# Stylish-TTS/stylish-tts

Hardware: AMD Instinct MI355X
Metric: audio frames/sec/GPU (24 kHz) forward+backward; DDP scaling 1/2/4/8 MI355X (higher is better)
Workload: dtype bf16 GEMM operands, f32 accumulation/storage; 1 GPU; c3: B=32/GPU T=520 frames (6.5 s) L=100

## Files before the change

include/stylish_hip.h:

```cpp
#ifndef STYLISH_HIP_H
#define STYLISH_HIP_H

#include <stddef.h>
#include <stdint.h>

#ifdef __cplusplus
extern "C" {
#endif

typedef enum {
  STY_OK = 0,
  STY_EINVAL = -1,
  STY_ESHAPE = -2,
  STY_EHIP = -3,
  STY_ENOMEM = -4,
  STY_ESTATE = -5
} sty_status;

typedef struct sty_model sty_model;

int sty_version(void);
const char *sty_last_error(void);

int sty_model_create(const char *kind, sty_model **out);
// ... 87 lines not shown
int sty_ctc_loss_fwd_bwd(int B, int T, int V1, int U, const float *log_probs, const float *log_priors, float prior_scale,
                         const int64_t *targets, const int64_t *input_lengths, const int64_t *target_lengths, int blank,
                         float weight, double *nll, float *loss, int32_t *status, float *d_logits, void *workspace,
                         size_t ws_bytes, void *stream);

int sty_convnext_fwd(sty_model *m, const char *prefix, int B, int C, int T, const float *x, const float *style,
                     float *y, void *workspace, size_t ws_bytes, void *stream);
int sty_resblock_fwd(sty_model *m, const char *prefix, int B, int T, const float *x, const float *style, float *y,
                     void *workspace, size_t ws_bytes, void *stream);
int sty_block_train_workspace_bytes(sty_model *m, const char *kind, const char *prefix, int B, int C, int T,
                                    size_t *bytes);
int sty_block_fwd_bwd(sty_model *m, const char *kind, const char *prefix, int B, int C, int T, const float *x,
                      const float *style, const float *gy, float *y, float *gx, float *d_style, void *workspace,
                      size_t ws_bytes, void *stream);
int sty_attention_workspace_bytes(int B, int H, int T, size_t *bytes);
int sty_attention_fwd_bwd(int B, int H, int DH, int T, const float *q, const float *k, const float *v,
                          const int64_t *lengths, const float *d_o, float *o, float *dq, float *dk, float *dv,
                          void *workspace, size_t ws_bytes, void *stream);
int sty_stft64_fwd(int B, int N, const float *wave, float *spec, float *phase, void *stream);
void sty_stft64_bases_host(float *out);
int sty_istft64_fwd(int B, int F, const float *logamp, const float *real, const float *imag, float *audio,
                    void *stream);
int sty_source_fwd(int B, int T, const float *pitch, const float *voiced, const float *noise, uint64_t seed,
                   const float *lin_w, const float *lin_b, float *prior, void *workspace, size_t ws_bytes,
                   void *stream);
int sty_source_workspace_bytes(int B, int T, size_t *bytes);
int sty_grn_bwd_workspace_bytes(int B, int C4, int T, size_t *bytes);
int sty_grn_bwd(int B, int C4, int T, const float *h, const float *ds, const float *gamma, int from_gx, float *coef,
                float *dgamma, void *workspace, size_t ws_bytes, void *stream);
int sty_act_bwd(int kind, int B, int C, int T, const float *x, float *dy, const float *alpha, const float *h,
                const float *coef, int fused, float *dx, int accumulate, float *dalpha, void *stream);
int sty_adain_finalize(int B, int C, int T, int nseg, const double *part, const float *gb, float eps, float *a, float *s,
                       float *mean, float *rstd, void *stream);

int sty_model_enable_training(sty_model *m);
typedef struct {
  int bn_batch_stats;
  int sn_power_iter;
  int f0_smooth;
  int energy_smooth;
  float bn_momentum;
  unsigned dropout_seed;
  float text_dropout;
  int compute_bf16;
  int frozen;
  float block_dropout;
} sty_train_opts;
int sty_model_set_train_opts(sty_model *m, const sty_train_opts *opts);

typedef void (*sty_grad_hook)(void *user, int segment);
int sty_model_set_grad_hook(sty_model *m, sty_grad_hook hook, void *user);
int sty_model_bind_grad(sty_model *m, const char *key, float *grad);
int sty_vocoder_train_workspace_bytes(sty_model *m, int B, int T, size_t *bytes);
int sty_vocoder_fwd_train(sty_model *m, const sty_vocoder_io *io, void *workspace, size_t ws_bytes, void *stream);
int sty_vocoder_bwd(sty_model *m, const float *d_audio, float *d_mel, float *d_style, void *stream);
int sty_speech_train_workspace_bytes(sty_model *m, int B, int L, int T, size_t *bytes);
int sty_speech_fwd_train(sty_model *m, const sty_speech_io *io, void *workspace, size_t ws_bytes, void *stream);
int sty_speech_bwd(sty_model *m, const float *d_audio, float *d_style, float *d_energy, void *stream);
int sty_speech_prepare_train(sty_model *m, void *stream);
int sty_speech_bwd_pe(sty_model *m, const float *d_audio, float *d_style, float *d_pitch, float *d_energy, void *stream);
int sty_speech_d_style_ready(sty_model *m, void *stream);
int sty_speech_branch_stream(sty_model *m, void **stream);
int sty_style_train_workspace_bytes(sty_model *m, int B, int T, size_t *bytes);
int sty_style_fwd_train(sty_model *m, int B, int T, const float *mel, float *style, void *workspace, size_t ws_bytes,
                        void *stream);
int sty_style_bwd(sty_model *m, const float *d_style, void *stream);
// ... 163 lines not shown
```

stylish_tts_amd/csrc/api.hip:

```cpp
#include <math.h>
#include <stdarg.h>
#include <string.h>
#include <stdlib.h>
#include <cxxabi.h>

#include <algorithm>
#include <functional>
#include <map>
#include <mutex>
#include <string>
#include <tuple>

#include "model.h"

namespace sty {

static thread_local char g_err[1024] = "";
void set_error(const char* fmt, ...) {
  va_list ap;
  va_start(ap, fmt);
  vsnprintf(g_err, sizeof(g_err), fmt, ap);
  va_end(ap);
}
int hip_fail(hipError_t e, const char* what) {
// ... 3380 lines not shown
  return launch_grn_bwd(from_gx ? gx : nullptr, part, nseg, gamma, ds, B, C4, coef, dgamma, st);
}
int sty_act_bwd(int kind, int B, int C, int T, const float* x, float* dy, const float* alpha, const float* h,
                const float* coef, int fused, float* dx, int accumulate, float* dalpha, void* stream) {
  if (!x || !dy || !dx || B <= 0 || C <= 0 || T <= 0 || (kind == ACT_SNAKE && !alpha) || ((h != nullptr) != (coef != nullptr))) {
    set_error("sty_act_bwd: bad argument");
    return STY_EINVAL;
  }
  hipStream_t st = S(stream);
  if (h && !fused) {
    const int rc = launch_row_scale_add(h, coef, 0.f, B * C, T, dy, st);
    if (rc) return rc;
    h = coef = nullptr;
  }
  if (deterministic_mode() && kind == ACT_SNAKE && dalpha && B > 1) {
    for (int b = 0; b < B; ++b) {
      const size_t o = (size_t)b * C * T;
      const int rc = launch_act_bwd(kind, x + o, dy + o, alpha, 1, C, T, dx + o, accumulate, dalpha, st, h ? h + o : nullptr,
                                    coef ? coef + (size_t)b * C : nullptr);
      if (rc) return rc;
    }
    return STY_OK;
  }
  return launch_act_bwd(kind, x, dy, alpha, B, C, T, dx, accumulate, dalpha, st, h, coef);
}
int sty_adain_finalize(int B, int C, int T, int nseg, const double* part, const float* gb, float eps, float* a, float* s,
                       float* mean, float* rstd, void* stream) {
  if (!part || !gb || !a || !s || B <= 0 || C <= 0 || T <= 0 || nseg <= 0 || ((mean != nullptr) != (rstd != nullptr))) {
    set_error("sty_adain_finalize: bad argument");
    return STY_EINVAL;
  }
  return launch_adain_finalize(part, nseg, gb, B, C, T, eps, a, s, S(stream), mean, rstd);
}
int sty_mel_workspace_bytes(int B, int N, int n_fft, int hop, size_t* bytes) {
  if (!bytes || B <= 0 || N <= n_fft / 2 || n_fft <= 0 || hop <= 0) {
    set_error("sty_mel_workspace_bytes: bad argument");
    return STY_EINVAL;
  }
  *bytes = mel_workspace_floats(B, N, n_fft, hop, 80) * sizeof(float);
  return STY_OK;
}
int sty_mel_fwd(int B, int N, const float* audio, int n_fft, int win_length, int hop, float mean, float std_,
                float* mel, float* energy, void* workspace, size_t ws_bytes, void* stream) {
  if (!audio || !mel || !workspace || B <= 0 || N <= n_fft / 2 || win_length > n_fft || hop <= 0 || std_ == 0.f) {
    set_error("sty_mel_fwd: bad argument");
    return STY_EINVAL;
  }
  if (ws_bytes < mel_workspace_floats(B, N, n_fft, hop, 80) * sizeof(float)) {
    set_error("sty_mel_fwd: workspace too small");
    return STY_ENOMEM;
  }
  return launch_mel(B, N, audio, n_fft, win_length, hop, 80, 24000, mean, std_, mel, energy, (float*)workspace,
                    S(stream));
}
int sty_multispec_workspace_bytes(int B, int N, size_t* bytes) {
  if (!bytes || B <= 0 || N <= 1024) {
    set_error("sty_multispec_workspace_bytes: bad argument");
    return STY_EINVAL;
  }
  size_t mx = 0;
  const int res[3][2] = {{512, 128}, {1024, 256}, {2048, 512}};
  for (auto& r : res) {
    const size_t n = multispec_workspace_floats(B, N, r[0], r[1]);
    mx = n > mx ? n : mx;
  }
  *bytes = mx * sizeof(float);
// ... 105 lines not shown
```

stylish_tts_amd/csrc/conv2d.hip:

```cpp
#include <stdlib.h>

#include "weights.h"

namespace sty {

constexpr int SN_SLICES = 8;
size_t sn_power_iter_scratch_floats(int Cout, int n) { return (size_t)SN_SLICES * n + Cout; }

int sn_wtu_blocks(int n) { return SN_SLICES * ((n + 255) / 256); }
__device__ __forceinline__ int snj_n(const SnPrepJob& j) { return j.depthwise ? 9 : j.Cin * j.KH * j.K; }
__global__ __launch_bounds__(256) void sn_wt_u_multi_kernel(const SnPrepJob* __restrict__ jobs, const int* __restrict__ job_of_blk) {
  const SnPrepJob j = jobs[job_of_blk[blockIdx.x]];
  const int n = snj_n(j), nib = (n + 255) / 256;
  const int local = (int)blockIdx.x - j.wtu0, slice = local / nib, i = (local - slice * nib) * 256 + threadIdx.x;
  if (i >= n) return;
  float s = 0.f;
  for (int co = slice; co < j.Cout; co += SN_SLICES) s = fmaf(j.w[(size_t)co * n + i], j.u[co], s);
  j.power[(size_t)slice * n + i] = s;
}
__global__ __launch_bounds__(256) void sn_normalize_multi_kernel(const SnPrepJob* __restrict__ jobs, int which) {
  __shared__ double red[256];
  const SnPrepJob j = jobs[blockIdx.x];
  const int nv = snj_n(j);
  const int n = which ? j.Cout : nv, slices = which ? 1 : SN_SLICES;
// ... 186 lines not shown
  return STY_OK;
}

__global__ __launch_bounds__(256) void dwconv2d_s2_kernel(const float* __restrict__ x, const float* __restrict__ w9,
                                                          const float* __restrict__ bias, int C, int H, int W, int Ho,
                                                          int Wo, float* __restrict__ y, __bf16* __restrict__ y16) {
  const int ldi = W + 1, ldo = Wo + 1;
  const int i = blockIdx.x * 256 + threadIdx.x;
  if (i >= Ho * ldo) return;
  const int ho = i / ldo, wo = i - ho * ldo;
  const int bc = blockIdx.y, c = bc % C;
  float* out = y + (size_t)bc * Ho * ldo + i;
  __bf16* out16 = y16 ? y16 + (size_t)bc * Ho * ldo + i : nullptr;
  if (wo == Wo) {
    *out = 0.f;
    if (out16) *out16 = (__bf16)0.f;
    return;
  }
  const float* p = x + (size_t)bc * H * ldi;
  float acc = bias[c];
#pragma unroll
  for (int kh = 0; kh < 3; ++kh) {
    const int hi = 2 * ho + kh - 1;
    if (hi < 0 || hi >= H) continue;
#pragma unroll
    for (int kw = 0; kw < 3; ++kw) {
      const int wi = 2 * wo + kw - 1;
      if (wi >= 0 && wi < W) acc = fmaf(w9[c * 9 + kh * 3 + kw], p[(size_t)hi * ldi + wi], acc);
    }
  }
  *out = acc;
  if (out16) *out16 = (__bf16)(acc < 0.f ? 0.2f * acc : acc);
}
int launch_dwconv2d_s2(const float* x, const float* w9, const float* bias, int B, int C, int H, int W, float* y,
                       hipStream_t st, __bf16* y16_lrelu) {
  const int Ho = (H - 1) / 2 + 1, Wo = (W - 1) / 2 + 1;
  hipLaunchKernelGGL(dwconv2d_s2_kernel, dim3(cdiv(Ho * (Wo + 1), 256), B * C), dim3(256), 0, st, x, w9, bias, C, H, W, Ho,
                     Wo, y, y16_lrelu);
  STY_LAUNCH_CHECK();
  return STY_OK;
}

__global__ __launch_bounds__(256) void avgpool2_kernel(const float* __restrict__ x, int H, int W, int Ho, int Wo,
                                                       float scale, float* __restrict__ y, __bf16* __restrict__ y16) {
  const int ldi = W + 1, ldo = Wo + 1;
  const int i = blockIdx.x * 256 + threadIdx.x;
  if (i >= Ho * ldo) return;
  const int ho = i / ldo, wo = i - ho * ldo;
  const int bc = blockIdx.y;
  float* out = y + (size_t)bc * Ho * ldo + i;
  __bf16* out16 = y16 ? y16 + (size_t)bc * Ho * ldo + i : nullptr;
  if (wo == Wo) {
    *out = 0.f;
    if (out16) *out16 = (__bf16)0.f;
    return;
  }
  const float* p = x + (size_t)bc * H * ldi;
  const int w0 = 2 * wo, w1 = min(2 * wo + 1, W - 1);
  const float s = p[(size_t)(2 * ho) * ldi + w0] + p[(size_t)(2 * ho) * ldi + w1] +
                  p[(size_t)(2 * ho + 1) * ldi + w0] + p[(size_t)(2 * ho + 1) * ldi + w1];
  *out = s * 0.25f * scale;
  if (out16) *out16 = (__bf16)(s * 0.25f * scale);
}
int launch_avgpool2(const float* x, int BC, int H, int W, float scale, float* y, hipStream_t st, __bf16* y16) {
  const int Ho = H / 2, Wo = (W + 1) / 2;
  hipLaunchKernelGGL(avgpool2_kernel, dim3(cdiv(Ho * (Wo + 1), 256), BC), dim3(256), 0, st, x, H, W, Ho, Wo, scale, y, y16);
  STY_LAUNCH_CHECK();
  return STY_OK;
}

__global__ __launch_bounds__(1024) void pool_fc_kernel(const float* __restrict__ x, int C, int n, float inv_count,
// ... 52 lines not shown
  const float* p = x + (size_t)bc * n;
  float* d = dx + (size_t)bc * n;
  __bf16* d16 = dx16 ? dx16 + (size_t)bc * n : nullptr;
  const float* mk = mask16 ? mask16 + (size_t)(bc / C) * n : nullptr;
  float wk[9];
#pragma unroll
  for (int k = 0; k < 9; ++k) wk[k] = w9[c * 9 + k];
  float wacc[10];
#pragma unroll
  for (int k = 0; k < 10; ++k) wacc[k] = 0.f;
  const int nq = Ho * Wo;
  auto put = [&](int o, float v) {
    if (ACC) v += d[o];
    if (ACC || dx) d[o] = v;
    if (!ACC && d16) d16[o] = (__bf16)(v * mk[o]);
  };
#pragma unroll 1
  for (int rr = 0; rr < DW2_R; ++rr) {
    const int q = (blockIdx.x * DW2_R + rr) * 256 + threadIdx.x;
    if (q >= nq) break;
    const int qh = q / Wo, qw = q - qh * Wo;
    const bool w1 = qw + 1 < Wo, h1 = qh + 1 < Ho;
    auto G = [&](int ho, int wo, bool ok) {
      if (!ok) return 0.f;
      float v = g[(size_t)ho * ldo + wo];
      if (gt && !(gt[(size_t)ho * ldo + wo] > 0.f)) v *= 0.2f;
      return v;
    };
    const float G00 = G(qh, qw, true), G01 = G(qh, qw + 1, w1), G10 = G(qh + 1, qw, h1), G11 = G(qh + 1, qw + 1, w1 && h1);
    const int hi = 2 * qh, wi = 2 * qw;
    const bool c1 = wi + 1 < W, r1 = hi + 1 < H;
    const int o0 = hi * ldi + wi, o1 = o0 + ldi;
    const float xee = p[o0], xeo = c1 ? p[o0 + 1] : 0.f, xoe = r1 ? p[o1] : 0.f, xoo = (c1 && r1) ? p[o1 + 1] : 0.f;
    put(o0, wk[4] * G00);
    wacc[4] = fmaf(G00, xee, wacc[4]);
    wacc[9] += G00;
    if (c1) {
      put(o0 + 1, fmaf(wk[3], G01, wk[5] * G00));
      wacc[3] = fmaf(G01, xeo, wacc[3]);
      wacc[5] = fmaf(G00, xeo, wacc[5]);
    }
    if (r1) {
      put(o1, fmaf(wk[1], G10, wk[7] * G00));
      wacc[1] = fmaf(G10, xoe, wacc[1]);
      wacc[7] = fmaf(G00, xoe, wacc[7]);
      if (c1) {
        put(o1 + 1, fmaf(wk[0], G11, fmaf(wk[2], G10, fmaf(wk[6], G01, wk[8] * G00))));
        wacc[0] = fmaf(G11, xoo, wacc[0]);
        wacc[2] = fmaf(G10, xoo, wacc[2]);
        wacc[6] = fmaf(G01, xoo, wacc[6]);
        wacc[8] = fmaf(G00, xoo, wacc[8]);
      }
    }
    if (qw == Wo - 1) {
      put(hi * ldi + W, 0.f);
      if (r1) put((hi + 1) * ldi + W, 0.f);
    }
  }
  const int lane = threadIdx.x & 63, wave = threadIdx.x >> 6;
#pragma unroll
  for (int k = 0; k < 10; ++k) {
    float v = wacc[k];
    for (int o = 32; o > 0; o >>= 1) v += __shfl_xor(v, o);
    if (lane == 0) red[wave][k] = v;
  }
  __syncthreads();
  if (threadIdx.x < 10) {
    const int k = threadIdx.x;
    part[((size_t)bc * gridDim.x + blockIdx.x) * 10 + k] = (red[0][k] + red[1][k]) + (red[2][k] + red[3][k]);
  }
}
__global__ __launch_bounds__(64) void dwconv2d_s2_bwd_w_sum_kernel(const float* __restrict__ part, int C, int B, int nblk,
                                                                   float* __restrict__ dw9, float* __restrict__ db) {
  const int c = blockIdx.x, lane = threadIdx.x;
  float s[10];
#pragma unroll
  for (int k = 0; k < 10; ++k) s[k] = 0.f;
  for (int b = 0; b < B; ++b) {
    const float* pp = part + ((size_t)(b * C + c) * nblk) * 10;
    for (int j = lane; j < nblk; j += 64)
#pragma unroll
      for (int k = 0; k < 10; ++k) s[k] += pp[(size_t)j * 10 + k];
  }
#pragma unroll
  for (int k = 0; k < 10; ++k) {
    float v = s[k];
    for (int o = 32; o > 0; o >>= 1) v += __shfl_xor(v, o);
    s[k] = v;
  }
  if (lane == 0) {
#pragma unroll
    for (int k = 0; k < 9; ++k) dw9[c * 9 + k] += s[k];
    if (db) db[c] += s[9];
  }
}
size_t dwconv2d_s2_bwd_scratch_floats(int B, int C, int H, int W) { return (size_t)B * C * cdiv(H * (W + 1), 1024) * 10; }
int launch_dwconv2d_s2_bwd(const float* x, const float* gy, const float* gate, const float* w9, int B, int C, int H, int W,
                           float* dx, int accumulate, float* dw9, float* db, float* scratch, hipStream_t st, __bf16* dx16,
                           const float* mask16) {
  const int Ho = (H - 1) / 2 + 1, Wo = (W - 1) / 2 + 1;
  const int nblk = cdiv(Ho * Wo, 256 * DW2_R);
  if (dx16 && (accumulate || !mask16)) {
    set_error("dwconv2d_s2_bwd: the operand twin of dx needs the overwriting form and the mask");
    return STY_EINVAL;
  }
  if (!dx && !dx16) {
    set_error("dwconv2d_s2_bwd: neither dx nor its operand twin to write");
    return STY_EINVAL;
  }
  if (accumulate)
    hipLaunchKernelGGL(dwconv2d_s2_bwd_kernel<true>, dim3(nblk, B * C), dim3(256), 0, st, x, gy, gate, w9, C, H, W, Ho, Wo, dx,
                       scratch, nullptr, nullptr);
  else
    hipLaunchKernelGGL(dwconv2d_s2_bwd_kernel<false>, dim3(nblk, B * C), dim3(256), 0, st, x, gy, gate, w9, C, H, W, Ho, Wo, dx,
                       scratch, dx16, mask16);
  hipLaunchKernelGGL(dwconv2d_s2_bwd_w_sum_kernel, dim3(C), dim3(64), 0, st, scratch, C, B, nblk, dw9, db);
  STY_LAUNCH_CHECK();
  return STY_OK;
}
__global__ void dw2d_sn_unpack_kernel(const float* __restrict__ g9, const float* __restrict__ w,
                                      const float* __restrict__ u, const float* __restrict__ v,
                                      const float* __restrict__ t, int C, float* __restrict__ dW) {
  __shared__ float red[2][256];
  float sig = 0.f, dot = 0.f;
  for (int i = threadIdx.x; i < C; i += 256) sig += t[i];
  for (int i = threadIdx.x; i < C * 9; i += 256) dot = fmaf(g9[i], w[i], dot);
  red[0][threadIdx.x] = sig;
  red[1][threadIdx.x] = dot;
  __syncthreads();
  for (int o = 128; o > 0; o >>= 1) {
    if (threadIdx.x < o) {
      red[0][threadIdx.x] += red[0][threadIdx.x + o];
      red[1][threadIdx.x] += red[1][threadIdx.x + o];
    }
    __syncthreads();
  }
  const float inv = 1.0f / red[0][0], k = red[1][0] * inv * inv;
  for (int i = threadIdx.x; i < C * 9; i += 256) dW[i] += g9[i] * inv - k * u[i / 9] * v[i % 9];
}
int launch_dw2d_sn_unpack(const float* g9, const float* w, const float* u, const float* v, const float* t, int C,
                          float* dW, hipStream_t st) {
  hipLaunchKernelGGL(dw2d_sn_unpack_kernel, dim3(1), dim3(256), 0, st, g9, w, u, v, t, C, dW);
  STY_LAUNCH_CHECK();
  return STY_OK;
}
__global__ __launch_bounds__(256) void avgpool2_bwd_kernel(const float* __restrict__ gy, int H, int W, int Ho, int Wo,
                                                           float scale, float* __restrict__ dx,
// ... 133 lines not shown
```

stylish_tts_amd/csrc/model.h:

```cpp
#pragma once
#include <math.h>

#include <map>
#include <string>
#include <unordered_map>
#include <vector>

#include "sty_common.h"
#include "weights.h"

namespace sty {

struct Param {
  const float* p = nullptr;
  std::vector<int64_t> shape;
};

int convnext32_ntiles(int T);
int launch_convnext32(const Cnx32Args& a, int B, int pass, hipStream_t st);
int launch_attention(const AttnArgs& a, int B, int DH, hipStream_t st);
int launch_rope_n(float* q, float* k, int B, int H, int DH, int L, int d, hipStream_t st, float sgn = 1.0f);
int launch_style_expand(const float* style, int B, int S, int L, float* y, hipStream_t st);
int launch_row_sum_add(const float* src, int rows, int L, float* dst, hipStream_t st);
int launch_wn_dw_bwd(const float* dw, const float* g, const float* v, int C, int K, float* dg, float* dv, hipStream_t st);
// ... 33 lines not shown
                 size_t ws_bytes, hipStream_t st, size_t* need);
struct AcousticGan {
  const sty_specdisc_params* p[3] = {nullptr, nullptr, nullptr};
  const sty_specdisc_grads* g[3] = {nullptr, nullptr, nullptr};
  float w_gen = 1.f, disc_scale = 1.f;
  float* out = nullptr;
  int bf16 = 0;
  void* ws = nullptr;
  size_t ws_bytes = 0;
};
size_t acoustic_gan_workspace_bytes(int B, int N, int with_grads);
int launch_acoustic_loss_gan(int B, int N, const float* audio_gt, const float* audio_pred, float w_mel, float w_phase,
                             float* losses_out, float* d_pred, float* ws, const AcousticGan* gan, hipStream_t st);
int launch_multispec_single(int B, int N, const float* audio, int n_fft, int hop, int sample_rate, float* mag,
                            float* phase, float* fft_mag, float* ws, hipStream_t st);
size_t loss_features_scratch_floats(int B, int N);
int launch_loss_features(int B, int N, const float* audio, int r, float* mag, float* scratch, hipStream_t st);

struct Bump {
  char* base = nullptr;
  size_t off = 0, cap = 0;
  bool overflow = false;
  template <typename T>
  T* take(size_t n) {
    off = align_up(off, 256);
    T* p = base ? reinterpret_cast<T*>(base + off) : nullptr;
    off += n * sizeof(T);
    if (base && off > cap) overflow = true;
    return p;
  }
};

int launch_dwconv2d_s2(const float* x, const float* w9, const float* bias, int B, int C, int H, int W, float* y,
                       hipStream_t st, __bf16* y16_lrelu = nullptr);
int launch_avgpool2(const float* x, int BC, int H, int W, float scale, float* y, hipStream_t st, __bf16* y16 = nullptr);
int launch_pool_fc(const float* x, int B, int C, int n, int count, const float* W, const float* bvec, int S,
                   float* out, hipStream_t st);
struct AdaFc {
  int idx = -1;
  int C = 0;
  size_t off = 0;
};

struct ConvNeXt {
  int C = 0;
  const float *dw_w = nullptr, *dw_b = nullptr, *b1 = nullptr, *alpha = nullptr, *grn_gamma = nullptr;
  AdaFc norm;
  PackedConv pw1, pw2;
  const float* w2a = nullptr;
  const float* w1p = nullptr;
  const float *w1_raw = nullptr, *w2_raw = nullptr;
};

struct ResBlock32 {
  PackedConv c1[3], c2[3];
  AdaFc n1[3], n2[3];
  const float *a1[3], *a2[3];
};

struct Conformer {
  AdaFc ff1n, ff2n, attn_n, conv_n, post_n;
  PackedConv ff1a, ff1b, ff2a, ff2b, to_q, to_kv, to_out, pw1, pw2;
  const float *dw_w, *dw_b, *bn_w, *bn_b, *bn_rm, *bn_rv;
};

struct VocoderPlan {
  PackedConv amp_input_conv;
// ... 271 lines not shown
int style_fc_bwd_slots(int nlayers);
int launch_istft64_bwd(int B, int F, const float* audio, const float* daudio, const float* logamp, const float* real,
                       const float* imag, const float* bbr, const float* bbi, float* dlogamp, float* dreal,
                       float* dimag, hipStream_t st);
size_t wgrad_partial_floats(const PackedConv& w, int B, int T);
struct WgReduceDefer;
WgReduceDefer* wgrad_defer_create();
void wgrad_defer_destroy(WgReduceDefer* d);
WgReduceDefer* wgrad_defer_set(WgReduceDefer* d);
size_t wgrad_defer_pending(const WgReduceDefer* d);
int wgrad_defer_flush(WgReduceDefer* d, int site, hipStream_t st);
void launch_wgrad_reduce_planes(const float* partial, int nslices, size_t plane, size_t stride, int nb, float* gwp,
                                float* gbias, hipStream_t st);
int launch_attention_bwd(const AttnArgs& a, const float* dO, float* dQ, float* dK, float* dV, size_t dqbs, size_t dkbs,
                         size_t dvbs, size_t dobs, int B, int DH, float* ws, hipStream_t st, int overwrite = 0);
bool attention_bwd_can_overwrite(const AttnArgs& a, int DH);
bool attention_bwd_mfma_dh(int DH);
size_t attention_bwd_ws_floats(int B, int H, int T);
int launch_rope_signed(float* q, float* k, int B, int H, int DH, int L, int d, const float* theta4, float sgn,
                       hipStream_t st);
int launch_embedding_bwd(const int64_t* tokens, const float* g, int B, int L, int H, int ntok, float scale, float* demb,
                         hipStream_t st, bool det = false);
int launch_bmm_ct_bwd(const float* g, const float* ali, int B, int C, int L, int T, float* denc, hipStream_t st);
int launch_slice_add(const float* src, int Csrc, int c0, int B, int C, int T, float* dst, hipStream_t st);
int launch_fnv_bwd(const float* pitch, const float* energy, const float* voiced, const float* w34, const float* g, int B,
                   int T, float* dw34, float* dp, float* de, float* dv, hipStream_t st, bool det = false);
int fnv_bwd_slices();
int launch_fnv_unpack(const float* dw34, const float* g0, const float* v0, const float* g1, const float* v1,
                      const float* g2, const float* v2, float* dg0, float* dv0, float* db0, float* dg1, float* dv1,
                      float* db1, float* dg2, float* dv2, float* db2, hipStream_t st);
size_t dwconv2d_s2_bwd_scratch_floats(int B, int C, int H, int W);
int launch_dwconv2d_s2_bwd(const float* x, const float* gy, const float* gate, const float* w9, int B, int C, int H, int W, float* dx,
                           int accumulate, float* dw9, float* db, float* scratch, hipStream_t st, __bf16* dx16 = nullptr,
                           const float* mask16 = nullptr);
int launch_pad_cols(const float* x, size_t rows, int W, float* y, hipStream_t st);
int launch_flat_mask(int B, int H, int Wp, int Hv, int Wv, float* m, hipStream_t st);
int launch_dw2d_sn_unpack(const float* g9, const float* w, const float* u, const float* v, const float* t, int C,
                          float* dW, hipStream_t st);
int launch_avgpool2_bwd(const float* gy, int BC, int H, int W, float scale, float* dx, const float* gate, hipStream_t st,
                        __bf16* dx16 = nullptr, const float* mask16 = nullptr, int C = 0);
int launch_pool_fc_bwd(const float* x, int B, int C, int n, int count, const float* W, int S, const float* gs,
                       float* dW, float* db, float* dx, int accumulate, hipStream_t st, float* det_a = nullptr);
int launch_bn_train_fwd(const float* x, const float* w, const float* b, float* rm, float* rv, float eps, float momentum,
                        int B, int C, int T, float* y, float* mean, float* rstd, double* part, hipStream_t st);
int launch_bn_train_bwd(const float* x, const float* dy, const float* w, const float* mean, const float* rstd, int B,
                        int C, int T, float* dx, int accumulate, float* dw, float* db, float* sums, hipStream_t st);
int launch_dropout(const float* x, const float* res, size_t n, float p, unsigned seed, unsigned site, float* y,
                   int accumulate, hipStream_t st, size_t group = 1);
int launch_box_smooth(const float* x, int B, int T, int width, float* y, int accumulate, hipStream_t st);
size_t sn_power_iter_scratch_floats(int Cout, int n);
int trainer_style_forward(struct Trainer* t, int B, int T, const float* mel, float* style, void* ws, size_t ws_bytes,
                          hipStream_t st, size_t* need, const float* pitch = nullptr, const float* energy = nullptr);
int trainer_style_backward(struct Trainer* t, const float* d_style, hipStream_t st);
int trainer_style_tap(struct Trainer* t, int i, int grad, float* dst, int* C, int* H, int* W, hipStream_t st);
inline sty_vocoder_io vocoder_io_of(const sty_speech_io& io) {
  sty_vocoder_io v = io.voc_taps;
  v.B = io.B;
  v.T = io.T;
  v.style = io.style;
  v.pitch = io.denormal_pitch;
  v.voiced = io.voiced;
  v.noise = io.noise;
  v.prior_override = io.prior_override;
  v.seed = io.seed;
  v.audio = io.audio;
  return v;
}
// ... 25 lines not shown
```

stylish_tts_amd/lib.py:

```python
import ctypes as C
import os

os.environ.setdefault("GPU_MAX_HW_QUEUES", "2")

HERE = os.path.dirname(os.path.abspath(__file__))
LIB_PATH = os.path.join(HERE, "libstylish_hip.so")


class StyError(RuntimeError):
    status = None


class StyDeviceError(StyError):
    """STY_EHIP: the HIP runtime reported an error (a failed launch, copy or allocation, a sticky device fault, no device).
    Not a refusal: nothing may be launched behind it, so nobody who skips refused work may catch it as one (`refused_on_host`)."""


STY_EHIP = -3


def refused_on_host(e):
    return isinstance(e, StyError) and not isinstance(e, StyDeviceError) and e.status != STY_EHIP


# ... 73 lines not shown
    "sty_model_set_train_opts": (C.c_int, [_P, C.POINTER(TrainOpts)]),
    "sty_vocoder_train_workspace_bytes": (C.c_int, [_P, _I, _I, _SZP]),
    "sty_vocoder_fwd_train": (C.c_int, [_P, C.POINTER(VocoderIO), _P, C.c_size_t, _P]),
    "sty_vocoder_bwd": (C.c_int, [_P, _P, _P, _P, _P]),
    "sty_speech_train_workspace_bytes": (C.c_int, [_P, _I, _I, _I, _SZP]),
    "sty_speech_fwd_train": (C.c_int, [_P, C.POINTER(SpeechIO), _P, C.c_size_t, _P]),
    "sty_speech_bwd": (C.c_int, [_P, _P, _P, _P, _P]),
    "sty_speech_prepare_train": (C.c_int, [_P, _P]),
    "sty_speech_bwd_pe": (C.c_int, [_P, _P, _P, _P, _P, _P]),
    "sty_speech_d_style_ready": (C.c_int, [_P, _P]),
    "sty_speech_branch_stream": (C.c_int, [_P, C.POINTER(C.c_void_p)]),
    "sty_style_train_workspace_bytes": (C.c_int, [_P, _I, _I, _SZP]),
    "sty_style_fwd_train": (C.c_int, [_P, _I, _I, _P, _P, _P, C.c_size_t, _P]),
    "sty_style_prepare_train": (C.c_int, [_P, _P]),
    "sty_style_bwd": (C.c_int, [_P, _P, _P]),
    "sty_style_tap": (C.c_int, [_P, _I, _I, _P, C.POINTER(C.c_int), C.POINTER(C.c_int), C.POINTER(C.c_int), _P]),
    "sty_duration_workspace_bytes": (C.c_int, [_P, _I, _I, _SZP]),
    "sty_duration_fwd": (C.c_int, [_P, _I, _I, _P, _P, _P, _P, _P, C.c_size_t, _P]),
    "sty_pitch_energy_workspace_bytes": (C.c_int, [_P, _I, _I, _I, _SZP]),
    "sty_pitch_energy_fwd": (C.c_int, [_P, _I, _I, _I, _P, _P, _P, _P, _P, _P, _P, C.c_size_t, _P]),
    "sty_pitch_style_workspace_bytes": (C.c_int, [_P, _I, _I, _SZP]),
    "sty_pitch_style_fwd": (C.c_int, [_P, _I, _I, _P, _P, _P, _P, _P, C.c_size_t, _P]),
    "sty_conv1d_workspace_bytes": (C.c_int, [_I, _I, _I, _SZP]),
    "sty_conv1d_fwd": (C.c_int, [_I, _I, _I, _I, _I, _I, _P, _P, _P, _P, _P, C.c_size_t, _I, _P]),
    "sty_conv1d_fwd_ex": (C.c_int, [_I, _I, _I, _I, _I, _I, _P, _P, _P, _P, _P, _P, _I, _I, _P, _P, C.c_size_t, _I, _P]),
    "sty_conv1d_route": (C.c_int, [_I, _I, _I, _I, _I, _I, _I, _I, C.POINTER(C.c_int)]),
    "sty_conv1d_bwd_workspace_bytes": (C.c_int, [_I, _I, _I, _I, _I, _SZP]),
    "sty_conv1d_bwd": (C.c_int, [_I, _I, _I, _I, _I, _I, _P, _P, _P, _P, _P, _P, _P, C.c_size_t, _I, _P]),
    "sty_partial_sum": (C.c_int, [_I, _P, _I, _I, _I, _P, _P, _P]),
    "sty_grn_bwd_workspace_bytes": (C.c_int, [_I, _I, _I, _SZP]),
    "sty_grn_bwd": (C.c_int, [_I, _I, _I, _P, _P, _P, _I, _P, _P, _P, C.c_size_t, _P]),
    "sty_act_bwd": (C.c_int, [_I, _I, _I, _I, _P, _P, _P, _P, _P, _I, _P, _I, _P, _P]),
    "sty_adain_finalize": (C.c_int, [_I, _I, _I, _I, _P, _P, C.c_float, _P, _P, _P, _P, _P]),
    "sty_adamw_step": (C.c_int, [C.c_size_t, _P, _P, _P, _P, C.c_float, C.c_float, C.c_float, C.c_float, C.c_float,
                                 _I, C.c_float, _P]),
    "sty_adamw_step_scaled": (C.c_int, [C.c_size_t, _P, _P, _P, _P, C.c_double, _P, C.c_float, C.c_float, C.c_float,
                                        C.c_float, _I, C.c_float, _P]),
    "sty_disc_lr_track": (C.c_int, [_P, _P, C.c_double, C.c_double, C.c_double, C.c_double, C.c_double, _P]),
    "sty_model_set_grad_hook": (C.c_int, [_P, _P, _P]),
    "sty_acoustic_loss_workspace_bytes": (C.c_int, [_I, _I, _SZP]),
    "sty_acoustic_loss_target": (C.c_int, [_I, _I, _P, _P, C.c_size_t, _P]),
    "sty_acoustic_loss_fwd_bwd": (C.c_int, [_I, _I, _P, _P, C.c_float, C.c_float, _P, _P, _P, C.c_size_t, _P]),
    "sty_mel_loss_workspace_bytes": (C.c_int, [_I, _I, _SZP]),
    "sty_mel_loss_features": (C.c_int, [_I, _I, _I, _I, _SZP, C.POINTER(C.c_int)]),
    "sty_mel_loss_fwd": (C.c_int, [_I, _I, _P, _P, _P, _P, _P, C.c_size_t, _P]),
    "sty_pitch_loss_fwd": (C.c_int, [_I, _I, _P, _P, _P, _P, C.c_size_t, _P]),
    "sty_duration_loss_fwd": (C.c_int, [_I, _I, _I, _P, _P, _P, _P, _P, _P, _P, _P, C.c_size_t, _P]),
    "sty_specdisc_workspace_bytes": (C.c_int, [_I, _I, _I, _I, _SZP]),
    "sty_specdisc_forward": (C.c_int, [_P, _I, _I, _I, _P, _P, _I, _P, C.c_size_t, _P]),
    "sty_specdisc_losses": (C.c_int, [_P, _I, _I, _I, _P, _P, C.c_float, _P, _P, C.c_float, _P, _P, _I, _P, C.c_size_t,
                                      _P]),
    "sty_prediction_to_duration": (C.c_int, [_I, _I, _I, _P, _P, _P, _P, _P]),
    "sty_duration_loss_fwd_bwd": (C.c_int, [_I, _I, _I, _P, _P, _P, _P, _P, _P, C.c_float, C.c_float, _P, _P, _P, _P,
                                            C.c_size_t, _P]),
    "sty_duration_train_workspace_bytes": (C.c_int, [_P, _I, _I, _SZP]),
    "sty_duration_fwd_train": (C.c_int, [_P, _I, _I, _P, _P, _P, _P, _P, C.c_size_t, _P]),
    "sty_duration_bwd": (C.c_int, [_P, _P, _P, _P]),
    "sty_pitch_loss_fwd_bwd": (C.c_int, [_I, _I, _P, _P, C.c_float, _I, _P, _P, _P, C.c_size_t, _P]),
    "sty_pitch_energy_train_workspace_bytes": (C.c_int, [_P, _I, _I, _I, _SZP]),
    "sty_pitch_energy_fwd_train": (C.c_int, [_P, _I, _I, _I, _P, _P, _P, _P, _P, _P, _P, C.c_size_t, _P]),
    "sty_pitch_energy_bwd": (C.c_int, [_P, _P, _P, _P, _P]),
    "sty_pitch_style_train_workspace_bytes": (C.c_int, [_P, _I, _I, _SZP]),
    "sty_pitch_style_fwd_train": (C.c_int, [_P, _I, _I, _P, _P, _P, _P, _P, C.c_size_t, _P]),
    "sty_pitchdisc_workspace_bytes": (C.c_int, [_I, _I, _I, _I, _I, _SZP]),
    "sty_pitchdisc_forward": (C.c_int, [_P, _I, _I, _I, _I, _P, _P, _P, C.c_size_t, _P]),
    "sty_pitchdisc_losses": (C.c_int, [_P, _I, _I, _I, _I, _P, _P, C.c_float, _P, _P, C.c_float, _P, _P, _P, C.c_size_t,
# ... 120 lines not shown
```

Baseline: 402,700 frames/s.

## Add LDS-staged wide kernels for stride-2 depthwise conv2d forward and backward

Adds new forward and backward kernels for the stride-2 3x3 depthwise conv2d. They stage the needed input (forward) or upstream gradient (backward) rows into shared memory with vectorized float4 loads, then have each thread produce four outputs with vector stores. The backward kernel walks the input grid (gather form), computes the weight-gradient partials alongside, and reduces them across waves. It also exposes the forward and backward as C API entry points with a 'present' flag that falls back to the old kernels, plus an env-var opt-out. The new path runs only when shapes and pointers meet alignment conditions, which adds branch complexity and the risk of subtle indexing errors at boundaries.

After: 406,500 frames/s, median of 6. About the same (+0.9%).

```diff
diff --git a/include/stylish_hip.h b/include/stylish_hip.h
--- a/include/stylish_hip.h
+++ b/include/stylish_hip.h
@@ -143,6 +143,12 @@
                 const float *coef, int fused, float *dx, int accumulate, float *dalpha, void *stream);
 int sty_adain_finalize(int B, int C, int T, int nseg, const double *part, const float *gb, float eps, float *a, float *s,
                        float *mean, float *rstd, void *stream);
+int sty_dwconv2d_s2_fwd(int B, int C, int H, int W, const float *x, const float *w9, const float *bias, float *y, void *y16,
+                        int present, void *stream);
+int sty_dwconv2d_s2_bwd_workspace_bytes(int B, int C, int H, int W, size_t *bytes);
+int sty_dwconv2d_s2_bwd(int B, int C, int H, int W, const float *x, const float *gy, const float *gate, const float *w9,
+                        float *dx, int accumulate, void *dx16, const float *mask16, float *dw9, float *db, void *workspace,
+                        size_t ws_bytes, int present, void *stream);
 
 int sty_model_enable_training(sty_model *m);
 typedef struct {
diff --git a/stylish_tts_amd/csrc/api.hip b/stylish_tts_amd/csrc/api.hip
--- a/stylish_tts_amd/csrc/api.hip
+++ b/stylish_tts_amd/csrc/api.hip
@@ -3436,6 +3436,36 @@
   }
   return launch_adain_finalize(part, nseg, gb, B, C, T, eps, a, s, S(stream), mean, rstd);
 }
+int sty_dwconv2d_s2_fwd(int B, int C, int H, int W, const float* x, const float* w9, const float* bias, float* y, void* y16,
+                        int present, void* stream) {
+  if (!x || !w9 || !bias || !y || B <= 0 || C <= 0 || H <= 0 || W <= 0) {
+    set_error("sty_dwconv2d_s2_fwd: bad argument");
+    return STY_EINVAL;
+  }
+  return launch_dwconv2d_s2(x, w9, bias, B, C, H, W, y, S(stream), reinterpret_cast<__bf16*>(y16), present != 0);
+}
+int sty_dwconv2d_s2_bwd_workspace_bytes(int B, int C, int H, int W, size_t* bytes) {
+  if (!bytes || B <= 0 || C <= 0 || H <= 0 || W <= 0) {
+    set_error("sty_dwconv2d_s2_bwd_workspace_bytes: bad argument");
+    return STY_EINVAL;
+  }
+  *bytes = dwconv2d_s2_bwd_scratch_floats(B, C, H, W) * sizeof(float);
+  return STY_OK;
+}
+int sty_dwconv2d_s2_bwd(int B, int C, int H, int W, const float* x, const float* gy, const float* gate, const float* w9,
+                        float* dx, int accumulate, void* dx16, const float* mask16, float* dw9, float* db, void* workspace,
+                        size_t ws_bytes, int present, void* stream) {
+  if (!x || !gy || !w9 || !dw9 || !workspace || B <= 0 || C <= 0 || H <= 0 || W <= 0 || (accumulate && !dx)) {
+    set_error("sty_dwconv2d_s2_bwd: bad argument");
+    return STY_EINVAL;
+  }
+  if (ws_bytes < dwconv2d_s2_bwd_scratch_floats(B, C, H, W) * sizeof(float)) {
+    set_error("sty_dwconv2d_s2_bwd: workspace too small");
+    return STY_ENOMEM;
+  }
+  return launch_dwconv2d_s2_bwd(x, gy, gate, w9, B, C, H, W, dx, accumulate, dw9, db, (float*)workspace, S(stream),
+                                reinterpret_cast<__bf16*>(dx16), mask16, present != 0);
+}
 int sty_mel_workspace_bytes(int B, int N, int n_fft, int hop, size_t* bytes) {
   if (!bytes || B <= 0 || N <= n_fft / 2 || n_fft <= 0 || hop <= 0) {
     set_error("sty_mel_workspace_bytes: bad argument");
diff --git a/stylish_tts_amd/csrc/conv2d.hip b/stylish_tts_amd/csrc/conv2d.hip
--- a/stylish_tts_amd/csrc/conv2d.hip
+++ b/stylish_tts_amd/csrc/conv2d.hip
@@ -242,11 +242,104 @@
   *out = acc;
   if (out16) *out16 = (__bf16)(acc < 0.f ? 0.2f * acc : acc);
 }
+constexpr int DW2W_LD = 8;
+constexpr int DW2W_CAP = DW2W_LD * 256 * 4;
+__device__ __forceinline__ int dw2w_sw8(int i) { return i + (i >> 3); }
+__global__ __launch_bounds__(256) void dwconv2d_s2_wide_kernel(const float* __restrict__ x, const float* __restrict__ w9,
+                                                               const float* __restrict__ bias, int C, int H, int W, int Ho,
+                                                               int Wo, int npb, float* __restrict__ y,
+                                                               __bf16* __restrict__ y16) {
+  __shared__ float xs[DW2W_CAP + DW2W_CAP / 8];
+  const int ldi = W + 1, ldo = Wo + 1, no = Ho * ldo;
+  const int bc = blockIdx.y, c = bc % C, tid = threadIdx.x;
+  const int o0 = blockIdx.x * npb, o1 = min(o0 + npb, no);
+  const int ho_lo = o0 / ldo, ho_hi = (o1 - 1) / ldo;
+  const int hi_lo = max(2 * ho_lo - 1, 0), hi_hi = min(2 * ho_hi + 1, H - 1);
+  const int s0 = (hi_lo * ldi) & ~3, s1 = ((hi_hi + 1) * ldi + 3) & ~3;
+  const float* p = x + (size_t)bc * H * ldi + s0;
+  float4 v[DW2W_LD];
+#pragma unroll
+  for (int k = 0; k < DW2W_LD; ++k) {
+    const int r = (k * 256 + tid) * 4;
+    v[k] = s0 + r < s1 ? *reinterpret_cast<const float4*>(p + r) : make_float4(0.f, 0.f, 0.f, 0.f);
+  }
+#pragma unroll
+  for (int k = 0; k < DW2W_LD; ++k) {
+    const int r = (k * 256 + tid) * 4;
+    if (s0 + r < s1) {
+      float* q = xs + dw2w_sw8(r);
+      q[0] = v[k].x;
+      q[1] = v[k].y;
+      q[2] = v[k].z;
+      q[3] = v[k].w;
+    }
+  }
+  __syncthreads();
+  const int o = o0 + tid * 4;
+  if (o >= o1) return;
+  float wk[9];
+#pragma unroll
+  for (int k = 0; k < 9; ++k) wk[k] = w9[c * 9 + k];
+  const float bv = bias[c];
+  int ho = o / ldo, wo = o - ho * ldo;
+  float out[4];
+#pragma unroll
+  for (int e = 0; e < 4; ++e) {
+    float acc = 0.f;
+    if (wo < Wo) {
+      const int rc = 2 * ho * ldi - s0 + 2 * wo;
+      const bool rt = ho > 0, rb = 2 * ho + 1 < H, cl = wo > 0, cr = 2 * wo + 1 < W;
+      acc = bv;
+#pragma unroll
+      for (int kh = 0; kh < 3; ++kh)
+#pragma unroll
+        for (int kw = 0; kw < 3; ++kw) {
+          const bool ok = (kh == 0 ? rt : kh == 2 ? rb : true) && (kw == 0 ? cl : kw == 2 ? cr : true);
+          const float xv = xs[dw2w_sw8(ok ? rc + (kh - 1) * ldi + (kw - 1) : rc)];
+          acc = ok ? fmaf(wk[kh * 3 + kw], xv, acc) : acc;
+        }
+    }
+    out[e] = acc;
+    if (++wo == ldo) {
+      wo = 0;
+      ++ho;
+    }
+  }
+  *reinterpret_cast<float4*>(y + (size_t)bc * no + o) = make_float4(out[0], out[1], out[2], out[3]);
+  if (y16) {
+    typedef __bf16 bf16x4 __attribute__((ext_vector_type(4)));
+    bf16x4 h;
+#pragma unroll
+    for (int e = 0; e < 4; ++e) h[e] = (__bf16)(out[e] < 0.f ? 0.2f * out[e] : out[e]);
+    *reinterpret_cast<bf16x4*>(y16 + (size_t)bc * no + o) = h;
+  }
+}
+static bool dw2_wide_off() { return getenv("STY_NO_DW2_WIDE") != nullptr; }
+static int dw2_wide_fwd_npb(int H, int W) {
+  const int Ho = (H - 1) / 2 + 1, Wo = (W - 1) / 2 + 1, ldi = W + 1, ldo = Wo + 1;
+  if ((H * ldi) % 4 || (Ho * ldo) % 4) return 0;
+  for (int npb = 1024; npb >= 256; npb /= 2) {
+    const int rows_o = std::min(Ho, (npb - 1 + ldo - 1) / ldo + 1);
+    const int rows_i = std::min(H, 2 * rows_o + 1);
+    if ((size_t)rows_i * ldi + 6 <= (size_t)DW2W_CAP) return npb;
+  }
+  return 0;
+}
 int launch_dwconv2d_s2(const float* x, const float* w9, const float* bias, int B, int C, int H, int W, float* y,
-                       hipStream_t st, __bf16* y16_lrelu) {
+                       hipStream_t st, __bf16* y16_lrelu, bool present) {
   const int Ho = (H - 1) / 2 + 1, Wo = (W - 1) / 2 + 1;
-  hipLaunchKernelGGL(dwconv2d_s2_kernel, dim3(cdiv(Ho * (Wo + 1), 256), B * C), dim3(256), 0, st, x, w9, bias, C, H, W, Ho,
-                     Wo, y, y16_lrelu);
+  const double ni = (double)B * C * H * (W + 1), no = (double)B * C * Ho * (Wo + 1);
+  const int npb = present || dw2_wide_off() || (((size_t)x | (size_t)y) & 15) || ((size_t)y16_lrelu & 7) ? 0 : dw2_wide_fwd_npb(H, W);
+  char detail[48];
+  snprintf(detail, sizeof(detail), "c%d h%d w%d", C, H, W);
+  ProfScope prof(npb ? "dwconv2d_s2_wide_kernel" : "dwconv2d_s2_kernel", 18.0 * no, 4.0 * ni + (y16_lrelu ? 6.0 : 4.0) * no, st,
+                 detail);
+  if (npb)
+    hipLaunchKernelGGL(dwconv2d_s2_wide_kernel, dim3(cdiv(Ho * (Wo + 1), npb), B * C), dim3(256), 0, st, x, w9, bias, C, H, W,
+                       Ho, Wo, npb, y, y16_lrelu);
+  else
+    hipLaunchKernelGGL(dwconv2d_s2_kernel, dim3(cdiv(Ho * (Wo + 1), 256), B * C), dim3(256), 0, st, x, w9, bias, C, H, W, Ho,
+                       Wo, y, y16_lrelu);
   STY_LAUNCH_CHECK();
   return STY_OK;
 }
@@ -365,7 +458,10 @@
     const bool c1 = wi + 1 < W, r1 = hi + 1 < H;
     const int o0 = hi * ldi + wi, o1 = o0 + ldi;
     const float xee = p[o0], xeo = c1 ? p[o0 + 1] : 0.f, xoe = r1 ? p[o1] : 0.f, xoo = (c1 && r1) ? p[o1 + 1] : 0.f;
-    put(o0, wk[4] * G00);
+    if (ACC)
+      d[o0] = fmaf(wk[4], G00, d[o0]);
+    else
+      put(o0, wk[4] * G00);
     wacc[4] = fmaf(G00, xee, wacc[4]);
     wacc[9] += G00;
     if (c1) {
@@ -427,12 +523,186 @@
     if (db) db[c] += s[9];
   }
 }
+constexpr int DW2W_CH = 4;
+constexpr int DW2W_NI = DW2W_CH * 256 * 4;
+constexpr int DW2W_GLD = 4;
+constexpr int DW2W_GCAP = DW2W_GLD * 256 * 4;
+__device__ __forceinline__ int dw2w_sw2(int i) { return i + (i >> 1); }
+__device__ __forceinline__ void dw2w_fmac(float& acc, float a, float b) { asm("v_fmac_f32 %0, %1, %2" : "+v"(acc) : "v"(a), "v"(b)); }
+__device__ __forceinline__ void dw2w_pin(float4& v) { asm volatile("" : "+v"(v.x), "+v"(v.y), "+v"(v.z), "+v"(v.w)); }
+template <bool ACC>
+__global__ __launch_bounds__(256) void dwconv2d_s2_bwd_wide_kernel(const float* __restrict__ x, const float* __restrict__ gy,
+                                                                   const float* __restrict__ gate,
+                                                                   const float* __restrict__ w9, int C, int H, int W, int Ho,
+                                                                   int Wo, float* __restrict__ dx, float* __restrict__ part,
+                                                                   __bf16* __restrict__ dx16,
+                                                                   const float* __restrict__ mask16) {
+  __shared__ float gs[DW2W_GCAP + DW2W_GCAP / 2];
+  __shared__ float red[4][10];
+  const int bc = blockIdx.y, c = bc % C, tid = threadIdx.x;
+  const int ldi = W + 1, ldo = Wo + 1, n = H * ldi;
+  const int i0 = blockIdx.x * DW2W_NI, i1 = min(i0 + DW2W_NI, n);
+  const int ho_lo = (i0 / ldi) >> 1, ho_hi = min((((i1 - 1) / ldi) >> 1) + 1, Ho - 1);
+  const int g0 = (ho_lo * ldo) & ~3, g1 = ((ho_hi + 1) * ldo + 3) & ~3;
+  const float* g = gy + (size_t)bc * Ho * ldo + g0;
+  const float* gt = gate ? gate + (size_t)bc * Ho * ldo + g0 : nullptr;
+  const float* p = x + (size_t)bc * n;
+  float* d = dx + (size_t)bc * n;
+  __bf16* d16 = dx16 ? dx16 + (size_t)bc * n : nullptr;
+  const float* mk = mask16 ? mask16 + (size_t)(bc / C) * n : nullptr;
+  const float4 zero4 = make_float4(0.f, 0.f, 0.f, 0.f);
+  float4 gv[DW2W_GLD], tv[DW2W_GLD], xv[DW2W_CH], mv[DW2W_CH], dv[DW2W_CH];
+#pragma unroll
+  for (int k = 0; k < DW2W_GLD; ++k) {
+    const int r = (k * 256 + tid) * 4, rc = g0 + r < g1 ? r : 0;
+    gv[k] = *reinterpret_cast<const float4*>(g + rc);
+    tv[k] = zero4;
+    if (gt) tv[k] = *reinterpret_cast<const float4*>(gt + rc);
+  }
+#pragma unroll
+  for (int j = 0; j < DW2W_CH; ++j) {
+    const int i = i0 + (j * 256 + tid) * 4, ic = i < i1 ? i : i0;
+    xv[j] = *reinterpret_cast<const float4*>(p + ic);
+    mv[j] = dv[j] = zero4;
+    if (!ACC && d16) mv[j] = *reinterpret_cast<const float4*>(mk + ic);
+    if (ACC) dv[j] = *reinterpret_cast<const float4*>(d + ic);
+  }
+#pragma unroll
+  for (int k = 0; k < DW2W_GLD; ++k) {
+    dw2w_pin(gv[k]);
+    dw2w_pin(tv[k]);
+  }
+#pragma unroll
+  for (int j = 0; j < DW2W_CH; ++j) {
+    dw2w_pin(xv[j]);
+    if (!ACC) dw2w_pin(mv[j]);
+    if (ACC) dw2w_pin(dv[j]);
+  }
+#pragma unroll
+  for (int k = 0; k < DW2W_GLD; ++k) {
+    const int r = (k * 256 + tid) * 4;
+    if (g0 + r < g1) {
+      float a[4] = {gv[k].x, gv[k].y, gv[k].z, gv[k].w};
+      if (gt) {
+        const float t[4] = {tv[k].x, tv[k].y, tv[k].z, tv[k].w};
+#pragma unroll
+        for (int e = 0; e < 4; ++e)
+          if (!(t[e] > 0.f)) a[e] *= 0.2f;
+      }
+      float* q = gs + dw2w_sw2(r);
+      q[0] = a[0];
+      q[1] = a[1];
+      q[3] = a[2];
+      q[4] = a[3];
+    }
+  }
+  __syncthreads();
+  float wk[9];
+#pragma unroll
+  for (int k = 0; k < 9; ++k) wk[k] = w9[c * 9 + k];
+  float wacc[10];
+#pragma unroll
+  for (int k = 0; k < 10; ++k) wacc[k] = 0.f;
+  const int step_h = 1024 / ldi, step_w = 1024 - step_h * ldi;
+  const int ibase = i0 + tid * 4;
+  int hc = ibase / ldi, wc = ibase - hc * ldi;
+#pragma unroll
+  for (int j = 0; j < DW2W_CH; ++j) {
+    const int i = ibase + j * 1024;
+    if (i < i1) {
+      int hi = hc, wi = wc;
+      int rowg = (hi >> 1) * ldo - g0;
+      const float xe[4] = {xv[j].x, xv[j].y, xv[j].z, xv[j].w};
+      const float me[4] = {mv[j].x, mv[j].y, mv[j].z, mv[j].w};
+      const float de[4] = {dv[j].x, dv[j].y, dv[j].z, dv[j].w};
+      float o32[4];
+      typedef __bf16 bf16x4 __attribute__((ext_vector_type(4)));
+      bf16x4 o16;
+#pragma unroll
+      for (int e = 0; e < 4; ++e) {
+        float v = 0.f;
+        if (wi < W) {
+          const int qh = hi >> 1, qw = wi >> 1;
+          const int gi = rowg + qw;
+          const bool w1 = qw + 1 < Wo, h1 = qh + 1 < Ho;
+          const float xx = xe[e];
+          const float G00 = gs[dw2w_sw2(gi)];
+          if (!(hi & 1)) {
+            if (!(wi & 1)) {
+              v = ACC ? fmaf(wk[4], G00, de[e]) : wk[4] * G00;
+              dw2w_fmac(wacc[4], G00, xx);
+              wacc[9] += G00;
+            } else {
+              const float t01 = gs[dw2w_sw2(w1 ? gi + 1 : gi)];
+              const float G01 = w1 ? t01 : 0.f;
+              v = fmaf(wk[3], G01, wk[5] * G00);
+              dw2w_fmac(wacc[3], G01, xx);
+              dw2w_fmac(wacc[5], G00, xx);
+            }
+          } else {
+            const float t10 = gs[dw2w_sw2(h1 ? gi + ldo : gi)];
+            const float G10 = h1 ? t10 : 0.f;
+            if (!(wi & 1)) {
+              v = fmaf(wk[1], G10, wk[7] * G00);
+              dw2w_fmac(wacc[1], G10, xx);
+              dw2w_fmac(wacc[7], G00, xx);
+            } else {
+              const float t01 = gs[dw2w_sw2(w1 ? gi + 1 : gi)];
+              const float t11 = gs[dw2w_sw2(w1 && h1 ? gi + ldo + 1 : gi)];
+              const float G01 = w1 ? t01 : 0.f, G11 = w1 && h1 ? t11 : 0.f;
+              v = fmaf(wk[0], G11, fmaf(wk[2], G10, fmaf(wk[6], G01, wk[8] * G00)));
+              dw2w_fmac(wacc[0], G11, xx);
+              dw2w_fmac(wacc[2], G10, xx);
+              dw2w_fmac(wacc[6], G01, xx);
+              dw2w_fmac(wacc[8], G00, xx);
+            }
+          }
+        }
+        if (ACC && !(wi < W && !(hi & 1) && !(wi & 1))) v += de[e];
+        o32[e] = v;
+        o16[e] = (__bf16)(v * me[e]);
+        if (++wi == ldi) {
+          wi = 0;
+          ++hi;
+          rowg = (hi >> 1) * ldo - g0;
+        }
+      }
+      if (ACC || dx) *reinterpret_cast<float4*>(d + i) = make_float4(o32[0], o32[1], o32[2], o32[3]);
+      if (!ACC && d16) *reinterpret_cast<bf16x4*>(d16 + i) = o16;
+    }
+    hc += step_h;
+    wc += step_w;
+    if (wc >= ldi) {
+      wc -= ldi;
+      ++hc;
+    }
+  }
+  const int lane = tid & 63, wave = tid >> 6;
+#pragma unroll
+  for (int k = 0; k < 10; ++k) {
+    float v = wacc[k];
+    for (int o = 32; o > 0; o >>= 1) v += __shfl_xor(v, o);
+    if (lane == 0) red[wave][k] = v;
+  }
+  __syncthreads();
+  if (tid < 10) part[((size_t)bc * gridDim.x + blockIdx.x) * 10 + tid] = (red[0][tid] + red[1][tid]) + (red[2][tid] + red[3][tid]);
+}
+static bool dw2_wide_bwd_fits(int H, int W) {
+  const int Ho = (H - 1) / 2 + 1, Wo = (W - 1) / 2 + 1, ldi = W + 1, ldo = Wo + 1;
+  if ((H * ldi) % 4 || (Ho * ldo) % 4) return false;
+  const int rows_i = std::min(H, (DW2W_NI - 1 + ldi - 1) / ldi + 1);
+  const int rows_o = std::min(Ho, rows_i / 2 + 2);
+  return (size_t)rows_o * ldo + 6 <= (size_t)DW2W_GCAP;
+}
+static_assert(DW2W_NI >= 1024, "dwconv2d_s2_bwd_scratch_floats sizes for at most one workgroup per 1024 input elements");
 size_t dwconv2d_s2_bwd_scratch_floats(int B, int C, int H, int W) { return (size_t)B * C * cdiv(H * (W + 1), 1024) * 10; }
 int launch_dwconv2d_s2_bwd(const float* x, const float* gy, const float* gate, const float* w9, int B, int C, int H, int W,
                            float* dx, int accumulate, float* dw9, float* db, float* scratch, hipStream_t st, __bf16* dx16,
-                           const float* mask16) {
+                           const float* mask16, bool present) {
   const int Ho = (H - 1) / 2 + 1, Wo = (W - 1) / 2 + 1;
-  const int nblk = cdiv(Ho * Wo, 256 * DW2_R);
+  const bool wide = !present && !dw2_wide_off() && dw2_wide_bwd_fits(H, W) &&
+                    !(((size_t)x | (size_t)gy | (size_t)gate | (size_t)dx | (size_t)mask16) & 15) && !((size_t)dx16 & 7);
+  const int nblk = wide ? cdiv(H * (W + 1), DW2W_NI) : cdiv(Ho * Wo, 256 * DW2_R);
   if (dx16 && (accumulate || !mask16)) {
     set_error("dwconv2d_s2_bwd: the operand twin of dx needs the overwriting form and the mask");
     return STY_EINVAL;
@@ -441,11 +711,23 @@
     set_error("dwconv2d_s2_bwd: neither dx nor its operand twin to write");
     return STY_EINVAL;
   }
-  if (accumulate)
-    hipLaunchKernelGGL(dwconv2d_s2_bwd_kernel<true>, dim3(nblk, B * C), dim3(256), 0, st, x, gy, gate, w9, C, H, W, Ho, Wo, dx,
+  const double ni = (double)B * C * H * (W + 1), no = (double)B * C * Ho * (Wo + 1);
+  char detail[48];
+  snprintf(detail, sizeof(detail), "c%d h%d w%d", C, H, W);
+  ProfScope prof(wide ? "dwconv2d_s2_bwd_wide_kernel" : "dwconv2d_s2_bwd_kernel", 27.0 * ni,
+                 ni * (4.0 + (accumulate ? 8.0 : dx ? 4.0 : 0.0) + (dx16 ? 2.0 : 0.0)) + no * (gate ? 8.0 : 4.0), st, detail);
+  const dim3 grid(nblk, B * C);
+  if (wide && accumulate)
+    hipLaunchKernelGGL(dwconv2d_s2_bwd_wide_kernel<true>, grid, dim3(256), 0, st, x, gy, gate, w9, C, H, W, Ho, Wo, dx, scratch,
+                       nullptr, nullptr);
+  else if (wide)
+    hipLaunchKernelGGL(dwconv2d_s2_bwd_wide_kernel<false>, grid, dim3(256), 0, st, x, gy, gate, w9, C, H, W, Ho, Wo, dx, scratch,
+                       dx16, mask16);
+  else if (accumulate)
+    hipLaunchKernelGGL(dwconv2d_s2_bwd_kernel<true>, grid, dim3(256), 0, st, x, gy, gate, w9, C, H, W, Ho, Wo, dx,
                        scratch, nullptr, nullptr);
   else
-    hipLaunchKernelGGL(dwconv2d_s2_bwd_kernel<false>, dim3(nblk, B * C), dim3(256), 0, st, x, gy, gate, w9, C, H, W, Ho, Wo, dx,
+    hipLaunchKernelGGL(dwconv2d_s2_bwd_kernel<false>, grid, dim3(256), 0, st, x, gy, gate, w9, C, H, W, Ho, Wo, dx,
                        scratch, dx16, mask16);
   hipLaunchKernelGGL(dwconv2d_s2_bwd_w_sum_kernel, dim3(C), dim3(64), 0, st, scratch, C, B, nblk, dw9, db);
   STY_LAUNCH_CHECK();
diff --git a/stylish_tts_amd/csrc/model.h b/stylish_tts_amd/csrc/model.h
--- a/stylish_tts_amd/csrc/model.h
+++ b/stylish_tts_amd/csrc/model.h
@@ -89,7 +89,7 @@
 };
 
 int launch_dwconv2d_s2(const float* x, const float* w9, const float* bias, int B, int C, int H, int W, float* y,
-                       hipStream_t st, __bf16* y16_lrelu = nullptr);
+                       hipStream_t st, __bf16* y16_lrelu = nullptr, bool present = false);
 int launch_avgpool2(const float* x, int BC, int H, int W, float scale, float* y, hipStream_t st, __bf16* y16 = nullptr);
 int launch_pool_fc(const float* x, int B, int C, int n, int count, const float* W, const float* bvec, int S,
                    float* out, hipStream_t st);
@@ -427,7 +427,7 @@
 size_t dwconv2d_s2_bwd_scratch_floats(int B, int C, int H, int W);
 int launch_dwconv2d_s2_bwd(const float* x, const float* gy, const float* gate, const float* w9, int B, int C, int H, int W, float* dx,
                            int accumulate, float* dw9, float* db, float* scratch, hipStream_t st, __bf16* dx16 = nullptr,
-                           const float* mask16 = nullptr);
+                           const float* mask16 = nullptr, bool present = false);
 int launch_pad_cols(const float* x, size_t rows, int W, float* y, hipStream_t st);
 int launch_flat_mask(int B, int H, int Wp, int Hv, int Wv, float* m, hipStream_t st);
 int launch_dw2d_sn_unpack(const float* g9, const float* w, const float* u, const float* v, const float* t, int C,
diff --git a/stylish_tts_amd/lib.py b/stylish_tts_amd/lib.py
--- a/stylish_tts_amd/lib.py
+++ b/stylish_tts_amd/lib.py
@@ -129,6 +129,9 @@
     "sty_grn_bwd": (C.c_int, [_I, _I, _I, _P, _P, _P, _I, _P, _P, _P, C.c_size_t, _P]),
     "sty_act_bwd": (C.c_int, [_I, _I, _I, _I, _P, _P, _P, _P, _P, _I, _P, _I, _P, _P]),
     "sty_adain_finalize": (C.c_int, [_I, _I, _I, _I, _P, _P, C.c_float, _P, _P, _P, _P, _P]),
+    "sty_dwconv2d_s2_fwd": (C.c_int, [_I, _I, _I, _I, _P, _P, _P, _P, _P, _I, _P]),
+    "sty_dwconv2d_s2_bwd_workspace_bytes": (C.c_int, [_I, _I, _I, _I, _SZP]),
+    "sty_dwconv2d_s2_bwd": (C.c_int, [_I, _I, _I, _I, _P, _P, _P, _P, _P, _I, _P, _P, _P, _P, _P, C.c_size_t, _I, _P]),
     "sty_adamw_step": (C.c_int, [C.c_size_t, _P, _P, _P, _P, C.c_float, C.c_float, C.c_float, C.c_float, C.c_float,
                                  _I, C.c_float, _P]),
     "sty_adamw_step_scaled": (C.c_int, [C.c_size_t, _P, _P, _P, _P, C.c_double, _P, C.c_float, C.c_float, C.c_float,
```
